# ivargr/kmer_mapper

Measured on AMD Instinct MI355X. Metric: M k-mers mapped/sec (whole node), k=31 150bp reads, higher is better.
Workload: dtype u64

## Files before the change

### kmer_mapper_amd/csrc/kmm.hip

```cpp
#include <hip/hip_runtime.h>

#include <cstdarg>
#include <cstdint>
#include <cstdio>
#include <cstdlib>
#include <chrono>
#include <cstring>
#include <memory>
#include <mutex>
#include <string>
#include <thread>
#include <utility>
#include <vector>

#include "kmm.h"

namespace {

thread_local std::string g_err;

int fail(int code, const char *fmt, ...)
{
    char buf[1024];
    va_list ap;
// ... 539 lines not shown
    if (w < 0 || w > 13 || ix->modulo >= (1ull << 31))
        return false;
    const uint64_t PF = (ix->modulo + (1ull << w) - 1) >> w;
    if (PF > (uint64_t)maxf * maxf)
        return false;
    int lg = 0;
    while ((1ull << lg) < PF)
        ++lg;
    int f2 = (lg + 1) / 2;
    bool for_filter = false;
    int occ_shift = 0;
    if (ix->rx_filter && w + f2 > P2F_LOGBITS) {
        const double load = ix->rx_S ? (double)ix->rx_S / (double)ix->modulo : 0.5;
        for (int gs = 0; gs <= 2 && !for_filter; ++gs) {
            const int fb = P2F_LOGBITS + gs - w;
            if (fb < 0 || load * (double)(1 << gs) > 0.75)
                continue;
            if (((PF + (1ull << fb) - 1) >> fb) <= (uint64_t)RX_MAXF && fb <= 9) {
                f2 = fb;
                occ_shift = gs;
                for_filter = true;
            }
        }
    }
    if (f2_force >= 0) {
        f2 = f2_force;
        occ_shift = w + f2 > P2F_LOGBITS ? w + f2 - P2F_LOGBITS : 0;
    }
    const uint64_t max_quo = ~0ull / ix->modulo;
    auto fits = [&](int sh) { return sh == 0 || (sh < 64 && (max_quo >> (64 - sh)) == 0); };
    while (f2 > 0 && !fits(w + f2))
        --f2;
    if (!fits(w + f2))
        return false;
    const uint64_t F2 = 1ull << f2, F1 = (PF + F2 - 1) / F2;
    if (F2 > (uint64_t)maxf || F1 > (uint64_t)(for_filter ? RX_MAXF : maxf))
        return false;
    ix->rx_w = w;
    ix->rx_f2 = f2;
    ix->rx_occ_shift = w + f2 > P2F_LOGBITS ? w + f2 - P2F_LOGBITS : 0;
    (void)occ_shift;
    ix->rx_PF = (uint32_t)PF;
    ix->rx_F1 = (uint32_t)F1;
    ix->rx_F2 = (uint32_t)F2;
    return true;
}

bool rx_filter_active(const kmm_index *ix)
{
    const int sh = ix->rx_w + ix->rx_f2;
    return ix->rx_filter && ix->rx_occ && sh - ix->rx_occ_shift >= 5 && ix->rx_occ_shift <= 2;
}

bool use_radix(const kmm_index *ix, int64_t units)
{
    if (!ix->rx_ok || ix->path == 1)
        return false;
    return ix->path == 2 || ix->rx_ecnt_acc || units >= ix->rx_min_units;
}

size_t align256(size_t x) { return (x + 255) & ~(size_t)255; }

template <int MODE>
int launch_rx(kmm_index *ix, const ReadsView &rv, const uint64_t *kmers_in, int64_t n_in, int k, int max_freq,
              int also_rc)
{
    const IndexView iv = view_of(ix);
    const int64_t units = MODE == MODE_KMERS ? n_in : rv.total;
    const int64_t n_src_total = MODE == MODE_PACKED ? (rv.n_reads + 2 * (int64_t)rv.pk_rpt - 1) / (2 * (int64_t)rv.pk_rpt)
                                                    : (units + RX_B - 1) / RX_B;
    const uint32_t X = also_rc ? 2u : 1u;
    const uint32_t F1 = ix->rx_F1, F2 = ix->rx_F2;
    int64_t n_sub = 1, max_src = 0;
    static const bool verbose = getenv("KMM_VERBOSE") != nullptr;
    const auto t_0 = std::chrono::steady_clock::now();
    if (ix->rx_sub_cap_eff > 0 && ++ix->rx_sub_cap_eff_age >= 16)
        ix->rx_sub_cap_eff = 0;
    int64_t cap = ix->rx_sub_cap_eff > 0 && ix->rx_sub_cap_eff < ix->rx_sub_cap ? ix->rx_sub_cap_eff : ix->rx_sub_cap;
    for (;;) {
        const int64_t cap_src = (cap / RX_B) / X > 0 ? (cap / RX_B) / X : 1;
        n_sub = (n_src_total + cap_src - 1) / cap_src;
        max_src = n_sub ? (n_src_total + n_sub - 1) / n_sub : cap_src;
        const size_t NBm = (size_t)max_src * X, chunks_m = (NBm + RX_CH - 1) / RX_CH, items_m = NBm + F1 + 1;
        const size_t meta = align256(NBm * (F1 + 1) * 2) + align256((size_t)F1 * (NBm + 1) * 4) + align256((size_t)F1 * NBm * 2) +
                            align256(chunks_m * F1 * 4) + 3 * align256((size_t)(F1 + 1) * 4) + align256(items_m * 8) +
                            align256(items_m * (F2 + 1) * 2) + align256(items_m * (F2 + 1) * 2 + 256) + align256(64) + align256(2048);
        int rc = ix->dbg_rx_buf_limit && NBm * RX_B * 8 > (size_t)ix->dbg_rx_buf_limit ? (int)KMM_ERR_NOMEM
                                                                                         : ensure(ix->rx_meta, meta);
        if (rc == KMM_OK)
            rc = ensure(ix->rx_buf1, NBm * RX_B * 8);
        if (rc == KMM_OK)
            rc = ensure(ix->rx_buf2, items_m * RX_B * 8);
        if (rc == KMM_OK)
            break;
        if (rc != KMM_ERR_NOMEM || cap <= ((int64_t)1 << 28) || n_src_total <= 1)
            return rc;
        (void)hipGetLastError();
        (void)ix->rx_buf1.reset();
        (void)ix->rx_buf2.reset();
        const int64_t next_src = (n_src_total + n_sub) / (n_sub + 1);
        cap = next_src * RX_B * X;
        if (cap < ((int64_t)1 << 28))
            cap = (int64_t)1 << 28;
        ix->rx_sub_cap_eff = cap;
        ix->rx_sub_cap_eff_age = 0;
    }
    ix->rx_sub_cap_last = cap;
    const double ms_buffers = ms_since(t_0);
    for (int64_t s0 = 0; s0 < n_src_total; s0 += max_src) {
        const uint32_t n_src = (uint32_t)(n_src_total - s0 < max_src ? n_src_total - s0 : max_src);
        const uint32_t NB = n_src * X;
        const uint32_t chunks = (NB + RX_CH - 1) / RX_CH;
        const size_t max_items = (size_t)NB + F1 + 1;
        RxView rx;
        memset(&rx, 0, sizeof rx);
        rx.pstart = ix->rx_pstart; rx.pkeys = ix->rx_pkeys; rx.pfreq = ix->rx_pfreq; rx.ecnt = ix->rx_ecnt;
        rx.pstart16 = ix->rx_pstart16; rx.slice_e0 = ix->rx_slice_e0; rx.slice_fmax = ix->rx_slice_fmax;
        rx.occ = ix->rx_occ;
        rx.occ_shift = rx_filter_active(ix) ? ix->rx_occ_shift : 3;
        rx.p2f_k = NB / 2048u < 4u ? 4u : (NB / 2048u > (uint32_t)P2F_KMAX ? (uint32_t)P2F_KMAX : NB / 2048u);
        rx.w = ix->rx_w; rx.f2 = ix->rx_f2; rx.PF = ix->rx_PF; rx.F1 = F1; rx.F2 = F2;
        rx.NB = NB; rx.max_items = (uint32_t)max_items;
        size_t off = 0;
        auto carve = [&](size_t bytes) { const size_t o = off; off += align256(bytes); return o; };
        const size_t o_start1 = carve((size_t)NB * (F1 + 1) * 2), o_P1T = carve((size_t)F1 * (NB + 1) * 4),
                     o_S1T = carve((size_t)F1 * NB * 2), o_csum = carve((size_t)chunks * F1 * 4),
                     o_T1 = carve((size_t)F1 * 4), o_ib = carve((size_t)(F1 + 1) * 4), o_wb = carve((size_t)(F1 + 1) * 4),
                     o_desc = carve(max_items * 8), o_start2 = carve(max_items * (F2 + 1) * 2), o_start2T = carve(max_items * (F2 + 1) * 2 + 256),
                     o_ctrl = carve(64),
                     o_queue = carve(2048);
        KMMCHK(ensure(ix->rx_meta, off));
        KMMCHK(ensure(ix->rx_buf1, (size_t)NB * RX_B * 8));
        KMMCHK(ensure(ix->rx_buf2, max_items * RX_B * 8));
        uint8_t *m = (uint8_t *)ix->rx_meta.p;
        rx.start1 = (uint16_t *)(m + o_start1); rx.P1T = (uint32_t *)(m + o_P1T); rx.S1T = (uint16_t *)(m + o_S1T);
        rx.csum = (uint32_t *)(m + o_csum); rx.T1 = (uint32_t *)(m + o_T1); rx.item_base = (uint32_t *)(m + o_ib);
        rx.work_base = (uint32_t *)(m + o_wb); rx.item_desc = (uint2 *)(m + o_desc);
        rx.start2 = (uint16_t *)(m + o_start2); rx.start2T = (uint16_t *)(m + o_start2T);
        rx.ctrl = (uint32_t *)(m + o_ctrl);
        rx.queue = (unsigned long long *)(m + o_queue);
        rx.buf1 = (uint64_t *)ix->rx_buf1.p;
        rx.buf2 = (uint64_t *)ix->rx_buf2.p;
#if RX_PROBE_ANY
        KMMCHK(ensure(ix->rx_probe, max_items * RX_B * 8));
        rx.probe = (uint64_t *)ix->rx_probe.p;
#endif
        ix->dbg_T1 = rx.T1; ix->dbg_item_base = rx.item_base; ix->dbg_start1 = rx.start1; ix->dbg_F1 = F1; ix->dbg_NB = NB;
        HIPCHK(hipMemsetAsync(m + o_ctrl, 0, align256(64) + 2048, ix->stream));
        ScopedTimer tm;
        KMMCHK(tm.begin(ix, KMM_KERNEL_RX_P1));
        static const int p1_per_cu = getenv("KMM_RX_P1_GRID_PER_CU") ? atoi(getenv("KMM_RX_P1_GRID_PER_CU")) : 8;
        const int64_t g1cap = (int64_t)ix->n_cu * (p1_per_cu > 0 ? p1_per_cu : 8);
        const dim3 g1((unsigned)(n_src < g1cap ? n_src : g1cap));
        const int64_t tile0 = s0 * (RX_B / (MODE == MODE_RECORDS ? 1024 : 4096));
        const uint64_t *src_kmers = kmers_in ? kmers_in + s0 * RX_B : nullptr;
        constexpr bool CAN_C2 = MODE == MODE_PACKED || MODE == MODE_UNIFORM || MODE == MODE_GENERAL;
        if (rv.codes2 && !CAN_C2)
            return fail(KMM_ERR_INTERNAL, "2-bit code input reaches pass 1 through the flat-read modes only");
        if constexpr (CAN_C2) {
            if (rv.codes2 && also_rc)
                hipLaunchKernelGGL((k_rx_p1<MODE, true, true>), g1, dim3(RX_NT), 0, ix->stream, rv, src_kmers, n_in - s0 * RX_B,
                                   iv, rx, k, tile0, n_src);
            else if (rv.codes2)
                hipLaunchKernelGGL((k_rx_p1<MODE, false, true>), g1, dim3(RX_NT), 0, ix->stream, rv, src_kmers, n_in - s0 * RX_B,
                                   iv, rx, k, tile0, n_src);
        }
        if (rv.codes2) {
        } else if (also_rc)
            hipLaunchKernelGGL((k_rx_p1<MODE, true>), g1, dim3(RX_NT), 0, ix->stream, rv, src_kmers, n_in - s0 * RX_B,
                               iv, rx, k, tile0, n_src);
        else
            hipLaunchKernelGGL((k_rx_p1<MODE, false>), g1, dim3(RX_NT), 0, ix->stream, rv, src_kmers, n_in - s0 * RX_B,
                               iv, rx, k, tile0, n_src);
        HIPCHK(hipGetLastError());
        KMMCHK(tm.end());
        KMMCHK(tm.begin(ix, KMM_KERNEL_RX_SCAN));
        hipLaunchKernelGGL(k_rx_colsum, dim3(chunks), dim3(256), 0, ix->stream, rx);
        hipLaunchKernelGGL(k_rx_chunkscan, dim3(F1), dim3(256), 0, ix->stream, rx, chunks);
        hipLaunchKernelGGL(k_rx_tables, dim3(1), dim3(512), 0, ix->stream, rx);
        hipLaunchKernelGGL(k_rx_colscan, dim3(chunks, (F1 + 255) / 256), dim3(256), 0, ix->stream, rx);
        HIPCHK(hipGetLastError());
        KMMCHK(tm.end());
        KMMCHK(tm.begin(ix, KMM_KERNEL_RX_P2));
        if (ix->rx_filter) {
            const bool flt = rx_filter_active(ix), small = F2 <= 128;
            auto kern = flt ? (small ? k_rx_p2f<true, true> : k_rx_p2f<true, false>)
                            : (small ? k_rx_p2f<false, true> : k_rx_p2f<false, false>);
            hipLaunchKernelGGL(kern, dim3(ix->n_cu), dim3(P2F_NT), 0, ix->stream, iv, rx);
        } else {
            hipLaunchKernelGGL(k_rx_p2, dim3(ix->n_cu * ix->rx_grid_per_cu), dim3(RX_NT), 0, ix->stream, iv, rx);
        }
        HIPCHK(hipGetLastError());
        KMMCHK(tm.end());
        KMMCHK(tm.begin(ix, KMM_KERNEL_RX_SCAN));
        hipLaunchKernelGGL(k_rx_tr2, dim3((unsigned)((max_items + RX_TR2 - 1) / RX_TR2)), dim3(256), 0, ix->stream, rx);
        HIPCHK(hipGetLastError());
        KMMCHK(tm.end());
        KMMCHK(tm.begin(ix, KMM_KERNEL_RX_P3));
        const bool p16 = ix->rx_pstart16 != nullptr;
        if (ix->rx_w > 12 && ix->rx_fits_small && p16)
            hipLaunchKernelGGL((k_rx_p3<RX_WMAX_BIG, RX_ECAP, 4, uint16_t, RX_SUBCAP3, true>), dim3(ix->n_cu * ix->rx_grid_per_cu),
                               dim3(RX_NT), 0, ix->stream, iv, rx, max_freq);
        else if (ix->rx_w > 12 && ix->rx_fits_small && ix->rx_max_slice <= 65535u)
            hipLaunchKernelGGL((k_rx_p3<RX_WMAX_BIG, RX_ECAP, 4, uint16_t>), dim3(ix->n_cu * ix->rx_grid_per_cu), dim3(RX_NT),
                               0, ix->stream, iv, rx, max_freq);
        else if (ix->rx_w > 12 && ix->rx_fits_mid && p16 && !getenv("KMM_RX_NO_MID"))
            hipLaunchKernelGGL((k_rx_p3<RX_WMAX_BIG, RX_ECAP_MID, 4, uint16_t, 1024, true>), dim3(ix->n_cu * ix->rx_grid_per_cu),
                               dim3(RX_NT), 0, ix->stream, iv, rx, max_freq);
        else if (ix->rx_w > 12 && ix->rx_fits_mid && ix->rx_max_slice <= 65535u && !getenv("KMM_RX_NO_MID"))
            hipLaunchKernelGGL((k_rx_p3<RX_WMAX_BIG, RX_ECAP_MID, 4, uint16_t, 1024>), dim3(ix->n_cu * ix->rx_grid_per_cu),
                               dim3(RX_NT), 0, ix->stream, iv, rx, max_freq);
        else if (ix->rx_w > 12)
            hipLaunchKernelGGL((k_rx_p3<RX_WMAX_BIG, RX_ECAP_BIG, 2, uint32_t>), dim3(ix->n_cu), dim3(RX_NT), 0, ix->stream,
                               iv, rx, max_freq);
        else if (ix->rx_w <= 12 && p16)
            hipLaunchKernelGGL((k_rx_p3<RX_WMAX, RX_ECAP, 4, uint16_t, RX_SUBCAP3, true>), dim3(ix->n_cu * ix->rx_grid_per_cu),
                               dim3(RX_NT), 0, ix->stream, iv, rx, max_freq);
        else
            hipLaunchKernelGGL((k_rx_p3<RX_WMAX, RX_ECAP, 4, uint32_t>), dim3(ix->n_cu * ix->rx_grid_per_cu), dim3(RX_NT), 0,
                               ix->stream, iv, rx, max_freq);
        HIPCHK(hipGetLastError());
        KMMCHK(tm.end());
        ix->ecnt_dirty = true;
        ix->rx_unchecked = true;
    }
    ix->n_radix_batches++;
    if (verbose && ms_since(t_0) > 20.0)
        fprintf(stderr, "libkmm: radix passes of %lld positions: %.2f ms for the batch buffers (%zu + %zu + %zu bytes), %.2f ms to issue %lld "
                "sub-batch(es)\n", (long long)units, ms_buffers, ix->rx_meta.cap, ix->rx_buf1.cap, ix->rx_buf2.cap, ms_since(t_0) - ms_buffers,
                (long long)n_sub);
    return KMM_OK;
}

int rx_flush(kmm_index *ix)
{
    if (!ix->ecnt_dirty)
        return KMM_OK;
    ScopedTimer tm;
    KMMCHK(tm.begin(ix, KMM_KERNEL_RX_FLUSH));
    if (ix->rx_norder && !ix->rx_ecnt_acc && ix->rx_flush_sorted) {
        hipLaunchKernelGGL(k_rx_flush_sorted, dim3(ix->n_cu * 8), dim3(256), 0, ix->stream, view_of(ix), ix->rx_ecnt,
                           ix->rx_norder, ix->rx_nnode, ix->rx_S);
        HIPCHK(hipMemsetAsync(ix->rx_ecnt, 0, (size_t)ix->rx_S * 4, ix->stream));
    } else {
        hipLaunchKernelGGL(k_rx_flush, dim3(ix->n_cu * 8), dim3(256), 0, ix->stream, view_of(ix), ix->rx_ecnt,
                           ix->rx_pnodes, ix->rx_S, ix->rx_ecnt_acc);
    }
    HIPCHK(hipGetLastError());
    KMMCHK(tm.end());
    ix->ecnt_dirty = false;
    return KMM_OK;
}

template <int MODE>
int launch_map_reads(kmm_index *ix, const ReadsView &rv, int k, int max_freq, int also_rc)
{
    const int64_t n_tiles = (rv.total + TILE_T - 1) / TILE_T;
    const bool radix = MODE == MODE_RECORDS ? false : use_radix(ix, rv.total);
    if (!radix) {
        KMMCHK(ensure_direct(ix));
        ix->n_direct_batches++;
        const IndexView iv = view_of(ix);
        ScopedTimer tm;
// ... 3329 lines not shown
```

### kmer_mapper_amd/csrc/kmm_radix.hpp

```cpp
#pragma once
#include <type_traits>

constexpr int RX_NT = 512;
constexpr int RX_B = 8192;
constexpr int RX_KPT = RX_B / RX_NT;
constexpr int RX_MAXF = 512;
#ifndef RX_CHV
#define RX_CHV 256
#endif
constexpr int RX_CH = RX_CHV;
constexpr int RX_IC = 1024;
#ifndef RX_LPR2V
#define RX_LPR2V 16
#endif
constexpr int RX_LPR = RX_LPR2V;
constexpr int RX_NG = RX_NT / RX_LPR;
#ifndef RX_RB1
#define RX_RB1 4
#endif
#ifndef RX_RB2
#define RX_RB2 8
#endif
constexpr int RX_SUBCAP = 1024;
#ifndef RX_SUBCAP3V
#define RX_SUBCAP3V 3072
#endif
constexpr int RX_SUBCAP3 = RX_SUBCAP3V;
#ifndef RX_LPR3
#define RX_LPR3 16
#endif
constexpr bool RX_P3_LINECUT = false;
constexpr int RX_LPR_P3 = RX_LPR3;
constexpr int RX_NG3 = RX_NT / RX_LPR_P3;
#ifndef RX_U3
#define RX_U3 8
#endif
constexpr int RX_U = RX_U3;
#ifndef RX_P3_GROUP
#define RX_P3_GROUP 4
#endif
constexpr int RX_G3 = RX_P3_GROUP;
#ifndef RX_U2V
#define RX_U2V 8
#endif
constexpr int RX_U2 = RX_U2V;
#ifdef RX_NT_LOADS
#define RX_LOAD2(p) __builtin_nontemporal_load(p)
#define RX_LOAD3(p) __builtin_nontemporal_load(p)
#else
#define RX_LOAD2(p) (*(p))
#define RX_LOAD3(p) (*(p))
#endif
constexpr int RX_WMAX = 4096;
constexpr int RX_ECAP = 4096;
constexpr int RX_WMAX_BIG = 8192;
constexpr int RX_ECAP_BIG = 8192;
constexpr int RX_ECAP_MID = 4608;
constexpr uint32_t RX_FILTERED = 0x80000000u;
enum { MODE_KMERS = 3 };

struct RxView {
    const uint16_t *pstart16;
    const uint32_t *slice_e0;
    const uint16_t *slice_fmax;
    const uint32_t *pstart;
    const uint64_t *pkeys;
    const uint16_t *pfreq;
    uint32_t *ecnt;
    const uint32_t *occ;
    uint32_t p2f_k;
    int w, f2;
    int occ_shift;
    uint32_t PF, F1, F2;
    uint32_t NB;
    uint32_t max_items;
    uint64_t *buf1, *buf2;
    uint16_t *start1;
    uint32_t *P1T;
    uint16_t *S1T;
    uint32_t *csum;
    uint32_t *T1;
    uint32_t *item_base;
    uint32_t *work_base;
    uint2 *item_desc;
    uint16_t *start2;
    uint16_t *start2T;
    uint32_t *ctrl;
    unsigned long long *queue;
    uint64_t *probe;
};

#ifndef RX_PROBE_P1W
#define RX_PROBE_P1W 0
#endif
#ifndef RX_PROBE_P2R
#define RX_PROBE_P2R 0
#endif
#ifndef RX_PROBE_P2W
#define RX_PROBE_P2W 0
#endif
#ifndef RX_PROBE_P3R
#define RX_PROBE_P3R 0
#endif
#define RX_PROBE_ANY (RX_PROBE_P1W || RX_PROBE_P2R || RX_PROBE_P2W || RX_PROBE_P3R)

__device__ __forceinline__ uint64_t rx_pack(const IndexView &iv, int sh, uint64_t q, uint32_t *coarse)
{
    uint32_t h;
    const uint64_t quo = fastdiv_m31(q, (uint32_t)iv.modulo, iv.magic, &h);
    *coarse = h >> sh;
    return (quo << sh) | (uint64_t)(h & ((1u << sh) - 1u));
}

__device__ __forceinline__ uint2 rx_pair(const uint32_t *s_in, int c0, int n)
{
    const uint2 p = *reinterpret_cast<const uint2 *>(s_in + c0);
    return make_uint2(c0 < n ? p.x : 0u, c0 + 1 < n ? p.y : 0u);
}

template <bool ONEBAR>
__device__ __forceinline__ uint32_t rx_scan256(const uint32_t *s_in, uint32_t *s_out, int n, uint32_t *s_wave, const int tid)
{
    if (ONEBAR) {
    (void)s_wave;
    const int lane = tid & 63;
    const int wave = __builtin_amdgcn_readfirstlane(tid >> 6);
    if (wave < 4) {
        const uint32_t v = tid < n ? s_in[tid] : 0u;
        const uint32_t inc = wave_scan_incl(v);
        uint32_t before = 0;
        for (int x = 0; x < wave; ++x) {
            const uint32_t t = x * 64 + lane < n ? s_in[x * 64 + lane] : 0u;
            before += (uint32_t)__builtin_amdgcn_readlane((int)wave_scan_incl(t), 63);
        }
        if (tid < n)
            s_out[tid] = before + inc - v;
        if (tid == 255)
            s_out[n] = before + inc;
    }
    __syncthreads();
    return s_out[n];
    }
    const int lane = tid & 63, wave = tid >> 6;
    const uint32_t v = tid < n ? s_in[tid] : 0u;
    const uint32_t inc = wave_scan_incl(v);
    if (wave < 4 && lane == 63)
        s_wave[wave] = inc;
    __syncthreads();
    const uint32_t total = s_wave[0] + s_wave[1] + s_wave[2] + s_wave[3];
    if (tid < n) {
        uint32_t base = 0;
        for (int x = 0; x < wave; ++x)
            base += s_wave[x];
        s_out[tid] = base + inc - v;
    }
    if (tid == 0)
        s_out[n] = total;
    __syncthreads();
    return total;
}
// ... 418 lines not shown
        lookups += (uint32_t)__popc(valid) * X;
        RX_PT(0);
        if (RC) {
            uint64_t x[RX_KPT];
            auto fwd = [&](int i) {
                uint32_t c;
                x[i] = rx_pack(iv, sh, q[i], &c);
                return ((valid >> i) & 1u) ? c : spare;
            };
            rx_sort_emit<RX_RB1, true, true, RX_NT, true, decltype(fwd), RxNoHook, 0, true>(
                x, fwd, F1, sbuf, s_cnt, s_base, s_wave, rx.buf1 + (size_t)sb * 2 * RX_B,
                rx.start1 + (size_t)sb * 2 * (size_t)(F1 + 1) RX_PT_ARG2, RxNoHook(), RX_KPT, wave_s);
            auto rev = [&](int i) {
                uint32_t c;
                x[i] = rx_pack(iv, sh, revcomp(q[i], k), &c);
                return ((valid >> i) & 1u) ? c : spare;
            };
            rx_sort_emit<RX_RB1, MODE == MODE_KMERS, true, RX_NT, true, decltype(rev), RxNoHook, 0, true>(
                x, rev, F1, sbuf, s_cnt, s_base, s_wave, rx.buf1 + ((size_t)sb * 2 + 1) * RX_B,
                rx.start1 + ((size_t)sb * 2 + 1) * (size_t)(F1 + 1) RX_PT_ARG2, RxNoHook(), RX_KPT, wave_s);
        } else {
            uint32_t qlo = 0, qhi = 0, rem = 0;
            const uint32_t M32 = (uint32_t)iv.modulo, Ml = M32 & 0xFFFFu, Mh = M32 >> 16;
            const uint32_t nb = (uint32_t)((win.lo >> (2 * k)) | (win.hi << (64 - 2 * k)));
            uint4 e_nx = make_uint4(0u, 0u, 0u, 0u);
            auto fwd = [&](int i) {
                if constexpr (INCDIV && R == 1) {
                    const uint4 e = e_nx;
                    if (i + 1 < RX_KPT) {
                        uint32_t c = (nb >> (2 * i)) & 3u;
                        asm("" : "+v"(c) : "v"(rem));
                        e_nx = s_qr[c];
                    }
                    if (i == 0) {
                        const uint64_t quot = fastdiv_m31(win.lo & tc.kmask, M32, iv.magic, &rem);
                        qlo = (uint32_t)quot;
                        qhi = (uint32_t)(quot >> 32);
                    } else {
                        const uint32_t t = qlo & 3u;
                        uint32_t th = __umul24(t, Mh);
                        asm("" : "+v"(th));
                        const uint32_t y = ((__umul24(t, Ml) + rem) >> 2) + (th << 14);
                        const uint32_t r2 = y + e.x;
                        uint32_t nlo, nhi;
                        asm("v_alignbit_b32 %0, %3, %2, 2\n\t"
                            "v_lshrrev_b32 %1, 2, %3\n\t"
                            "v_cmp_le_u32 vcc, %6, %7\n\t"
                            "v_addc_co_u32 %0, vcc, %0, %4, vcc\n\t"
                            "v_addc_co_u32 %1, vcc, %1, %5, vcc"
                            : "=&v"(nlo), "=&v"(nhi)
                            : "v"(qlo), "v"(qhi), "v"(e.y), "v"(e.z), "s"(M32), "v"(r2)
                            : "vcc");
                        qlo = nlo;
                        qhi = nhi;
                        rem = r2 - M32 < r2 ? r2 - M32 : r2;
                    }
                    q[i] = ((((uint64_t)qhi << 32) | qlo) << sh) | (uint64_t)(rem & ((1u << sh) - 1u));
                    return ((valid >> i) & 1u) ? rem >> sh : spare;
                } else {
                    uint32_t c;
                    q[i] = rx_pack(iv, sh, q[i], &c);
                    return ((valid >> i) & 1u) ? c : spare;
                }
            };
            auto post = [&]() {
                if constexpr (STAGE_EARLY) {
                    if (sb + sb_step < sb_end)
                        tile_packed_stage<C2>(rv, tile_begin + ((int64_t)(sb + sb_step) * 2 + half), sm[half], ltid, pw[0]);
                }
            };
            rx_sort_emit<RX_RB1, MODE == MODE_KMERS, true, RX_NT, true, decltype(fwd), RxNoHook, 0, true, decltype(post)>(
                q, fwd, F1, sbuf, s_cnt, s_base, s_wave, rx.buf1 + (size_t)sb * RX_B,
                rx.start1 + (size_t)sb * (size_t)(F1 + 1) RX_PT_ARG2, RxNoHook(), RX_KPT, wave_s, post,
                RX_PROBE_P1W ? rx.probe + (size_t)sb * RX_B : nullptr, RX_PROBE_P1W);
        }
    }
#ifdef RX_PT_P1
    RX_PT_END(iv, 10);
#endif
    rx_stat_add(iv, 0, lookups);
    rx_stat_add(iv, KMM_STAT_RX_P1, lookups);
}

__global__ void __launch_bounds__(256) k_rx_colsum(RxView rx)
{
    const uint32_t F1 = rx.F1;
    const uint32_t b0 = blockIdx.x * RX_CH;
    const uint32_t b1 = b0 + RX_CH < rx.NB ? b0 + RX_CH : rx.NB;
    const size_t ld = F1 + 1;
    for (uint32_t c = threadIdx.x; c < F1; c += 256) {
        const uint16_t *p = rx.start1 + (size_t)b0 * ld + c;
        uint32_t sum = 0, b = b0;
        for (; b + 8 <= b1; b += 8, p += 8 * ld) {
            uint32_t lo[8], hi[8];
#pragma unroll
            for (int u = 0; u < 8; ++u) {
                lo[u] = p[u * ld];
                hi[u] = p[u * ld + 1];
            }
#pragma unroll
            for (int u = 0; u < 8; ++u)
                sum += hi[u] - lo[u];
        }
        for (; b < b1; ++b, p += ld)
            sum += (uint32_t)p[1] - (uint32_t)p[0];
        rx.csum[(size_t)blockIdx.x * F1 + c] = sum;
    }
}

__device__ __forceinline__ uint32_t scan256_excl(uint32_t v, uint32_t *s_wave4, uint32_t *total)
{
    const int lane = threadIdx.x & 63, wave = threadIdx.x >> 6;
    const uint32_t inc = wave_scan_incl(v);
    __syncthreads();
    if (lane == 63)
        s_wave4[wave] = inc;
    __syncthreads();
    uint32_t base = 0;
    for (int x = 0; x < wave; ++x)
        base += s_wave4[x];
    *total = s_wave4[0] + s_wave4[1] + s_wave4[2] + s_wave4[3];
    return base + inc - v;
}

__global__ void __launch_bounds__(256) k_rx_chunkscan(RxView rx, uint32_t n_chunks)
{
    __shared__ uint32_t s_wave4[4];
    const uint32_t c = blockIdx.x, F1 = rx.F1;
    uint32_t carry = 0;
    for (uint32_t base = 0; base < n_chunks; base += 256) {
        const uint32_t ch = base + threadIdx.x;
        const uint32_t v = ch < n_chunks ? rx.csum[(size_t)ch * F1 + c] : 0u;
        uint32_t tot;
        const uint32_t ex = scan256_excl(v, s_wave4, &tot);
        if (ch < n_chunks)
            rx.csum[(size_t)ch * F1 + c] = carry + ex;
        carry += tot;
    }
    if (threadIdx.x == 0) {
        rx.T1[c] = carry;
        rx.P1T[(size_t)c * (rx.NB + 1) + rx.NB] = carry;
    }
}

__device__ __forceinline__ uint32_t scan512_excl(uint32_t v, uint32_t *s_wave8, uint32_t *total)
{
    const int lane = threadIdx.x & 63, wave = threadIdx.x >> 6;
    const uint32_t inc = wave_scan_incl(v);
    __syncthreads();
    if (lane == 63)
        s_wave8[wave] = inc;
    __syncthreads();
    uint32_t base = 0, tot = 0;
    for (int x = 0; x < 8; ++x) {
        base += x < wave ? s_wave8[x] : 0u;
        tot += s_wave8[x];
    }
    *total = tot;
    return base + inc - v;
}

__global__ void __launch_bounds__(512) k_rx_tables(RxView rx)
{
    static_assert(RX_MAXF <= 512, "one thread per coarse partition");
    __shared__ uint32_t s_wave8[8];
    const uint32_t c = threadIdx.x, F1 = rx.F1;
    const uint32_t run = c < F1 ? rx.T1[c] : 0u;
    const uint32_t n_items = c < F1 ? (run + RX_B - 1) / RX_B : 0u;
    const uint32_t rows = (n_items + RX_IC - 1) / RX_IC;
    uint32_t tot_items, tot_rows;
    const uint32_t ib = scan512_excl(n_items, s_wave8, &tot_items);
    const uint32_t wb = scan512_excl(rows, s_wave8, &tot_rows);
    uint32_t jmax = n_items;
#pragma unroll
    for (int d = 32; d > 0; d >>= 1) {
        const uint32_t o = __shfl_xor(jmax, d);
        jmax = o > jmax ? o : jmax;
    }
    __syncthreads();
    if ((threadIdx.x & 63) == 0)
        s_wave8[threadIdx.x >> 6] = jmax;
    __syncthreads();
    if (c < F1) {
        rx.item_base[c] = ib;
        rx.work_base[c] = wb;
    }
    if (c == 0) {
        uint32_t m = s_wave8[0];
        for (int x = 1; x < 8; ++x)
            m = s_wave8[x] > m ? s_wave8[x] : m;
        rx.item_base[F1] = tot_items;
        rx.work_base[F1] = tot_rows;
        rx.ctrl[0] = tot_items;
        rx.ctrl[1] = tot_rows;
        rx.ctrl[2] = m;
    }
}

__global__ void __launch_bounds__(256) k_rx_colscan(RxView rx)
{
    constexpr int TB = 32, CW = 256;
    __shared__ uint32_t tP[CW][TB + 1];
    __shared__ uint16_t tS[CW][TB + 2];
    const uint32_t F1 = rx.F1, NB = rx.NB;
    const uint32_t b0 = blockIdx.x * RX_CH;
    const uint32_t b1 = b0 + RX_CH < NB ? b0 + RX_CH : NB;
    const size_t ld = F1 + 1;
    const uint32_t lane = threadIdx.x & 63, wave = threadIdx.x >> 6;
    {
    const uint32_t cb = blockIdx.y * CW;
    const uint32_t c = cb + threadIdx.x;
    const uint32_t nc = F1 - cb < (uint32_t)CW ? F1 - cb : (uint32_t)CW;
    uint32_t run = c < F1 ? rx.csum[(size_t)blockIdx.x * F1 + c] : 0u;
    const uint32_t ib = c < F1 ? rx.item_base[c] : 0u;
    for (uint32_t t0 = b0; t0 < b1; t0 += TB) {
        const uint32_t nb = b1 - t0 < (uint32_t)TB ? b1 - t0 : (uint32_t)TB;
        if (c < F1) {
            const uint16_t *p = rx.start1 + (size_t)t0 * ld + c;
            uint32_t lo[TB], hi[TB];
#pragma unroll
            for (int u = 0; u < TB; ++u) {
                lo[u] = (uint32_t)u < nb ? p[u * ld] : 0u;
                hi[u] = (uint32_t)u < nb ? p[u * ld + 1] : 0u;
            }
#pragma unroll
            for (int u = 0; u < TB; ++u) {
                const uint32_t cnt = hi[u] - lo[u];
                tP[threadIdx.x][u] = run;
                tS[threadIdx.x][u] = (uint16_t)lo[u];
                if (cnt) {
                    uint32_t m = (run + RX_B - 1) / RX_B;
                    while ((uint64_t)m * RX_B < (uint64_t)run + cnt) {
                        rx.item_desc[ib + m] = make_uint2(t0 + u, c);
                        ++m;
                    }
                }
                run += cnt;
            }
        }
        __syncthreads();
        const uint32_t bi = lane & 31;
        for (uint32_t cc = wave * 2 + (lane >> 5); cc < nc; cc += 8) {
            if (bi < nb) {
                rx.P1T[(size_t)(cb + cc) * (NB + 1) + t0 + bi] = tP[cc][bi];
                rx.S1T[(size_t)(cb + cc) * NB + t0 + bi] = tS[cc][bi];
            }
        }
        __syncthreads();
    }
    }
}

constexpr int RX_TR2 = 32;
__global__ void __launch_bounds__(256) k_rx_tr2(RxView rx)
{
    __shared__ uint16_t tile[RX_TR2][RX_MAXF + 2];
    const uint32_t n_items = rx.ctrl[0], cols = rx.F2 + 1;
    const uint32_t i0 = blockIdx.x * RX_TR2;
    if (i0 >= n_items)
        return;
    const uint32_t ni = n_items - i0 < (uint32_t)RX_TR2 ? n_items - i0 : (uint32_t)RX_TR2;
    for (uint32_t e = threadIdx.x; e < ni * cols; e += 256)
        tile[e / cols][e % cols] = rx.start2[(size_t)i0 * cols + e];
    __syncthreads();
    const uint32_t it = threadIdx.x % RX_TR2, c0 = threadIdx.x / RX_TR2;
    if (it < ni)
        for (uint32_t col = c0; col < cols; col += 256 / RX_TR2)
            rx.start2T[(size_t)col * rx.max_items + i0 + it] = tile[it][col];
}

__global__ void __launch_bounds__(RX_NT, 4) k_rx_p2(IndexView iv, RxView rx)
{
    __shared__ uint64_t sbuf[RX_B];
    __shared__ uint32_t sub_src[RX_SUBCAP];
    __shared__ uint32_t sub_meta[RX_SUBCAP], s_wave8[2][RX_NT / 64];
    __shared__ __attribute__((aligned(8))) uint32_t s_cnt[RX_MAXF + 2 + 64];
    __shared__ uint32_t s_base[RX_MAXF + 1], s_wave[4];
    __shared__ uint32_t s_idx;
    const int tid = threadIdx.x, grp = tid / RX_LPR, lg = tid % RX_LPR;
    const uint32_t NB = rx.NB;
    uint32_t gathered = 0;
    uint32_t scan_flip = 0;
    const uint32_t spare = rx_spare_key();
    const int F2 = (int)rx.F2;
    const uint32_t cs = (rx.F1 + 7u) / 8u, limit = rx.ctrl[2] * cs;
    const uint32_t home = rx_xcc_id();
    if (tid <= F2)
        s_cnt[tid] = 0;
    if (tid == 0)
        s_cnt[RX_NT] = 0;
    struct Item {
        uint32_t valid, c, item, b0, lo, hi;
    };
    struct RunDesc {
        uint32_t vs, ve, st;
    };
    auto describe = [&](uint32_t sub, uint32_t idx) {
        Item d;
        d.valid = 0; d.c = 0; d.item = 0; d.b0 = 0; d.lo = 0; d.hi = 0;
        if (idx >= limit)
            return d;
        const uint32_t cj = idx / cs, cc = sub * cs + idx % cs;
        if (cc >= rx.F1)
            return d;
        const uint32_t ib = rx.item_base[cc];
        if (cj >= rx.item_base[cc + 1] - ib)
            return d;
        d.valid = 1;
        d.c = cc;
        d.item = ib + cj;
        d.b0 = rx.item_desc[d.item].x;
        d.lo = cj * RX_B;
        const uint32_t Tc = rx.T1[cc];
        d.hi = Tc - d.lo < (uint32_t)RX_B ? Tc : d.lo + RX_B;
        return d;
    };
    auto run_desc = [&](const Item &d, uint32_t bb) {
        RunDesc r;
        r.vs = 0xFFFFFFFFu; r.ve = 0xFFFFFFFFu; r.st = 0;
        const uint32_t b = bb + tid;
        if (d.valid && b < NB) {
            const uint32_t *P = rx.P1T + (size_t)d.c * (NB + 1);
            r.vs = P[b];
            r.ve = P[b + 1];
            r.st = rx.S1T[(size_t)d.c * NB + b];
        }
        return r;
    };
    RX_PT_DECL;
    for (uint32_t turn = 0; turn < 8u; ++turn) {
    const uint32_t sub = (home + turn) & 7u;
    uint32_t nxt = limit;
    if (tid == 0)
        nxt = rx_pop(rx.queue, sub, limit);
    if (tid == 0)
        s_idx = nxt;
    __syncthreads();
    uint32_t idx = s_idx;
    __syncthreads();
    if (idx >= limit)
        continue;
    if (tid == 0)
        nxt = rx_pop(rx.queue, sub, limit);
    Item it = describe(sub, idx);
    RunDesc rd = run_desc(it, it.b0);
    for (;;) {
        RX_PT(0);
        const uint32_t lo = it.lo, hi = it.hi, n = hi - lo;
        if (it.valid) {
            for (uint32_t bb = it.b0;; bb += RX_NT) {
                if (bb != it.b0)
                    rd = run_desc(it, bb);
                const uint32_t b = bb + tid;
                const uint32_t vs = rd.vs < hi ? rd.vs : hi;
                const bool live = vs < hi;
                const uint32_t ve = live ? rd.ve : vs;
                const uint32_t st = live ? rd.st : 0u;
                const uint32_t from = vs > lo ? vs : lo, to = ve < hi ? ve : hi;
                const uint32_t len = live && to > from ? to - from : 0u;
                const uint64_t src = (uint64_t)b * RX_B + st + (from - vs);
                uint32_t n_sub;
                const uint32_t last_more = (tid == RX_NT - 1 && live && ve < hi) ? 0x80000000u : 0u;
                const uint32_t pre = rx_scan_threads(rx_n_pieces<RX_LPR, true>(len, src) | last_more, s_wave8, scan_flip, &n_sub);
                const bool more = n_sub >> 31;
                n_sub &= 0x7FFFFFFFu;
                RX_PT(1);
                for (uint32_t win = 0; win < n_sub; win += RX_SUBCAP) {
                    rx_list_subruns<RX_LPR, true>(pre, len, src, from - lo, win, sub_src, sub_meta);
                    const uint32_t nw = n_sub - win < (uint32_t)RX_SUBCAP ? n_sub - win : (uint32_t)RX_SUBCAP;
                    rx_pad_list<RX_NG * RX_U2>(nw, sub_src, sub_meta);
                    __syncthreads();
                    for (uint32_t j0 = grp; j0 < nw; j0 += RX_NG * RX_U2) {
                        uint64_t x[RX_U2];
                        uint32_t meta[RX_U2], so[RX_U2];
#pragma unroll
                        for (int u = 0; u < RX_U2; ++u) {
                            meta[u] = sub_meta[j0 + u * RX_NG];
                            so[u] = sub_src[j0 + u * RX_NG];
                        }
#pragma unroll
                        for (int u = 0; u < RX_U2; ++u) {
                            const uint32_t rel = (uint32_t)lg - ((meta[u] >> 6) & 63u);
                            x[u] = rel < (meta[u] & 63u) ? RX_LOAD2(rx.buf1 + ((size_t)so[u] + lg)) : 0ull;
                        }
#pragma unroll
                        for (int u = 0; u < RX_U2; ++u) {
                            const uint32_t rel = (uint32_t)lg - ((meta[u] >> 6) & 63u);
                            if (rel < (meta[u] & 63u))
                                sbuf[(meta[u] >> 12) + rel] = x[u];
                        }
                    }
                    if (more || win + RX_SUBCAP < n_sub)
                        __syncthreads();
                }
                if (!more)
                    break;
            }
        }
        if (tid == 0)
            s_idx = nxt;
        __syncthreads();
        const uint32_t idx_n = s_idx;
        if (tid == 0 && idx_n < limit)
            nxt = rx_pop(rx.queue, sub, limit);
        const Item it_n = describe(sub, idx_n);
        RunDesc rd_n;
        rd_n.vs = 0xFFFFFFFFu; rd_n.ve = 0xFFFFFFFFu; rd_n.st = 0;
        if (it.valid) {
// ... 29 lines not shown
    }
#ifndef RX_PT_P1
    RX_PT_END(iv, 10);
#endif
    rx_stat_add(iv, 2, gathered);
}

__device__ __forceinline__ uint32_t rx_fold2(uint32_t x)
{
    x = (x | (x >> 1)) & 0x55555555u;
    x = (x | (x >> 1)) & 0x33333333u;
    x = (x | (x >> 2)) & 0x0F0F0F0Fu;
    x = (x | (x >> 4)) & 0x00FF00FFu;
    return (x | (x >> 8)) & 0x0000FFFFu;
}
__device__ __forceinline__ uint32_t rx_fold4(uint32_t x)
{
    x = (x | (x >> 1) | (x >> 2) | (x >> 3)) & 0x11111111u;
    x = (x | (x >> 3)) & 0x03030303u;
    x = (x | (x >> 6)) & 0x000F000Fu;
    return (x | (x >> 12)) & 0xFFu;
}

constexpr int P2F_NT = 1024;
constexpr int P2F_KPT = RX_B / P2F_NT;
constexpr int P2F_KMAX = 64;
constexpr int P2F_LOGBITS = 19;

template <bool FILTER, bool FSMALL>
__global__ void __launch_bounds__(P2F_NT) k_rx_p2f(IndexView iv, RxView rx)
{
    __shared__ uint32_t s_bits[(1 << P2F_LOGBITS) / 32];
    __shared__ uint64_t sbuf[RX_B];
    __shared__ uint32_t t_vs[P2F_NT + 64];
    __shared__ uint32_t t_off[P2F_NT];
    __shared__ uint16_t t_aux[RX_B / 64 + 1];
    __shared__ uint32_t t_last;
    __shared__ uint32_t t_sbits[2][RX_B / 32];
    __shared__ uint32_t t_empty[2];
    __shared__ __attribute__((aligned(8))) uint32_t s_cnt2[2][RX_MAXF + 2 + 64];
    __shared__ uint32_t s_base[RX_MAXF + 1], s_wave[4];
    __shared__ uint32_t s_b0[P2F_KMAX];
    __shared__ uint32_t s_idx;
    const int tid = threadIdx.x, lane = tid & 63;
    const uint32_t wave = (uint32_t)__builtin_amdgcn_readfirstlane(tid >> 6);
    const uint32_t NB = rx.NB;
    const int F2 = (int)rx.F2, w = rx.w;
    const uint32_t bmask = (1u << (rx.w + rx.f2)) - 1u;
    const uint32_t gs = (uint32_t)rx.occ_shift;
    constexpr bool nofilt = !FILTER;
    const uint32_t nwords = nofilt ? 0u : (((uint32_t)F2 << w) >> gs) / 32u;
    const uint32_t spare = rx_spare_key();
    uint32_t gathered = 0, dropped = 0;
    const uint32_t cs = (rx.F1 + 7u) / 8u;
    const uint32_t P2F_K = rx.p2f_k;
    const uint32_t limit = ((rx.ctrl[2] + P2F_K - 1u) / P2F_K) * cs;
    const uint32_t home = rx_xcc_id();
    if (tid <= F2)
        s_cnt2[0][tid] = s_cnt2[1][tid] = 0;
    RX_PT_DECL;

    struct RunDesc {
        uint32_t vs, ve, st;
    };
    for (uint32_t turn = 0; turn < 8u; ++turn) {
    const uint32_t sub = (home + turn) & 7u;
    for (;;) {
        if (tid == 0)
            s_idx = rx_pop(rx.queue, sub, limit);
        __syncthreads();
        const uint32_t idx = s_idx;
        __syncthreads();
        if (idx >= limit)
            break;
        const uint32_t cu = idx / cs, cc = sub * cs + idx % cs;
        if (cc >= rx.F1)
            continue;
        const uint32_t ib = rx.item_base[cc], n_items_c = rx.item_base[cc + 1] - ib;
        if (cu * P2F_K >= n_items_c)
            continue;
        const uint32_t j0 = cu * P2F_K;
        const uint32_t n_it = n_items_c - j0 < P2F_K ? n_items_c - j0 : P2F_K;
        const uint32_t Tc = rx.T1[cc];
        const uint32_t *P = rx.P1T + (size_t)cc * (NB + 1);
        const uint16_t *S = rx.S1T + (size_t)cc * NB;
        if ((uint32_t)tid < n_it)
            s_b0[tid] = rx.item_desc[ib + j0 + tid].x;
        if (nofilt) {
        } else if (gs == 0) {
            const uint4 *src = reinterpret_cast<const uint4 *>(rx.occ + (size_t)cc * nwords);
            uint4 *dst = reinterpret_cast<uint4 *>(s_bits);
            for (uint32_t i = tid; i < nwords / 4u; i += P2F_NT)
                dst[i] = src[i];
            for (uint32_t i = (nwords & ~3u) + tid; i < nwords; i += P2F_NT)
                s_bits[i] = rx.occ[(size_t)cc * nwords + i];
        } else {
            const uint32_t *src = rx.occ + (((size_t)cc * nwords) << gs);
            for (uint32_t i = tid; i < nwords; i += P2F_NT) {
                uint32_t o = 0;
                if (gs == 1) {
                    const uint2 v = *reinterpret_cast<const uint2 *>(src + 2 * (size_t)i);
                    o = rx_fold2(v.x) | (rx_fold2(v.y) << 16);
                } else {
                    const uint4 v = *reinterpret_cast<const uint4 *>(src + 4 * (size_t)i);
                    o = rx_fold4(v.x) | (rx_fold4(v.y) << 8) | (rx_fold4(v.z) << 16) | (rx_fold4(v.w) << 24);
                }
                s_bits[i] = o;
            }
        }
        if (tid < 2 * (RX_B / 32))
            (&t_sbits[0][0])[tid] = 0u;
        if (tid < 2)
            t_empty[tid] = 0u;
        __syncthreads();

        auto item_lo = [&](uint32_t j) { return (j0 + j) * (uint32_t)RX_B; };
        auto item_n = [&](uint32_t j) {
            const uint32_t lo = (j0 + j) * (uint32_t)RX_B;
            return Tc - lo < (uint32_t)RX_B ? Tc - lo : (uint32_t)RX_B;
        };
        auto load_desc = [&](uint32_t bb) {
            RunDesc r;
            const uint32_t b = bb + tid;
            r.vs = 0xFFFFFFFFu; r.ve = 0xFFFFFFFFu; r.st = 0;
            if (b < NB) {
                r.vs = P[b];
                r.ve = P[b + 1];
                r.st = S[b];
            }
            return r;
        };
        auto put_table = [&](const RunDesc &r, uint32_t lo, uint32_t hi, int mb = -1) {
            if (mb >= 0 && r.vs != 0xFFFFFFFFu && r.vs > lo && r.vs < hi) {
                if (r.ve > r.vs)
                    atomicOr(&t_sbits[mb][(r.vs - lo) >> 5], 1u << ((r.vs - lo) & 31u));
                else
                    t_empty[mb] = 1u;
            }
            t_vs[tid] = r.vs;
            t_off[tid] = (uint32_t)tid * RX_B + r.st - r.vs;
            if (tid == P2F_NT - 1) {
                t_vs[P2F_NT] = r.ve;
                if (r.ve < hi)
                    t_last = P2F_NT - 1;
            }
            const uint32_t from = r.vs > lo ? r.vs : lo, to = r.ve < hi ? r.ve : hi;
            if (r.vs != 0xFFFFFFFFu && from < to) {
                for (uint32_t a = (from - lo + 63u) >> 6; lo + (a << 6) < to; ++a)
                    t_aux[a] = (uint16_t)tid;
                if (to == hi)
                    t_last = (uint32_t)tid;
            }
        };
        auto fill = [&](auto merge_tag, uint32_t bb, uint32_t lo, uint32_t n, uint32_t c_lo, uint32_t c_hi,
                        uint64_t (&x)[P2F_KPT], int mb = -1) {
            constexpr bool MERGE = decltype(merge_tag)::value;
            const uint32_t c_end = lo + n < c_hi ? lo + n : c_hi;
            const uint32_t a0 = wave * 8u;
            uint32_t av = 0;
            {
                const uint32_t pa = lo + ((a0 + (uint32_t)lane) << 6);
                const uint32_t ia = a0 + ((uint32_t)lane <= 8u ? (uint32_t)lane : 8u);
                const uint32_t aux = t_aux[ia];
                av = pa < c_lo ? 0u : (pa < c_end ? aux : t_last);
            }
            uint32_t A[P2F_KPT + 1];
#pragma unroll
            for (int i = 0; i <= P2F_KPT; ++i)
// ... 721 lines not shown
```

Before: 169,600.

## Restructure radix column-scan with 64x64 tiles and padded transposed tables

Pads the transposed P1T/S1T tables to a leading dimension rounded up to 64 so that tiled writes start line-aligned. Rewrites k_rx_colscan to process 64-column by 64-row tiles with four waves that split the rows, software-prefetch the next tile, derive counts through a lane shuffle instead of a second load, and scan across waves through shared memory. k_rx_colsum now loads each start1 entry once and differences adjacent columns through shared memory, launched with one thread per column. The goal is to cut redundant global loads and uncoalesced stores in the scan stage. The cost is more shared-memory synchronisation and slightly larger metadata buffers.

```diff
diff --git a/kmer_mapper_amd/csrc/kmm.hip b/kmer_mapper_amd/csrc/kmm.hip
--- a/kmer_mapper_amd/csrc/kmm.hip
+++ b/kmer_mapper_amd/csrc/kmm.hip
@@ -645,7 +645,8 @@
         n_sub = (n_src_total + cap_src - 1) / cap_src;
         max_src = n_sub ? (n_src_total + n_sub - 1) / n_sub : cap_src;
         const size_t NBm = (size_t)max_src * X, chunks_m = (NBm + RX_CH - 1) / RX_CH, items_m = NBm + F1 + 1;
-        const size_t meta = align256(NBm * (F1 + 1) * 2) + align256((size_t)F1 * (NBm + 1) * 4) + align256((size_t)F1 * NBm * 2) +
+        const size_t ldTm = (NBm + RX_TT) / RX_TT * RX_TT;
+        const size_t meta = align256(NBm * (F1 + 1) * 2) + align256((size_t)F1 * ldTm * 4) + align256((size_t)F1 * ldTm * 2) +
                             align256(chunks_m * F1 * 4) + 3 * align256((size_t)(F1 + 1) * 4) + align256(items_m * 8) +
                             align256(items_m * (F2 + 1) * 2) + align256(items_m * (F2 + 1) * 2 + 256) + align256(64) + align256(2048);
         int rc = ix->dbg_rx_buf_limit && NBm * RX_B * 8 > (size_t)ix->dbg_rx_buf_limit ? (int)KMM_ERR_NOMEM
@@ -684,10 +685,11 @@
         rx.p2f_k = NB / 2048u < 4u ? 4u : (NB / 2048u > (uint32_t)P2F_KMAX ? (uint32_t)P2F_KMAX : NB / 2048u);
         rx.w = ix->rx_w; rx.f2 = ix->rx_f2; rx.PF = ix->rx_PF; rx.F1 = F1; rx.F2 = F2;
         rx.NB = NB; rx.max_items = (uint32_t)max_items;
+        rx.ldT = (NB + RX_TT) / RX_TT * RX_TT;
         size_t off = 0;
         auto carve = [&](size_t bytes) { const size_t o = off; off += align256(bytes); return o; };
-        const size_t o_start1 = carve((size_t)NB * (F1 + 1) * 2), o_P1T = carve((size_t)F1 * (NB + 1) * 4),
-                     o_S1T = carve((size_t)F1 * NB * 2), o_csum = carve((size_t)chunks * F1 * 4),
+        const size_t o_start1 = carve((size_t)NB * (F1 + 1) * 2), o_P1T = carve((size_t)F1 * rx.ldT * 4),
+                     o_S1T = carve((size_t)F1 * rx.ldT * 2), o_csum = carve((size_t)chunks * F1 * 4),
                      o_T1 = carve((size_t)F1 * 4), o_ib = carve((size_t)(F1 + 1) * 4), o_wb = carve((size_t)(F1 + 1) * 4),
                      o_desc = carve(max_items * 8), o_start2 = carve(max_items * (F2 + 1) * 2), o_start2T = carve(max_items * (F2 + 1) * 2 + 256),
                      o_ctrl = carve(64),
@@ -738,10 +740,10 @@
         HIPCHK(hipGetLastError());
         KMMCHK(tm.end());
         KMMCHK(tm.begin(ix, KMM_KERNEL_RX_SCAN));
-        hipLaunchKernelGGL(k_rx_colsum, dim3(chunks), dim3(256), 0, ix->stream, rx);
+        hipLaunchKernelGGL(k_rx_colsum, dim3(chunks), dim3((F1 + 63) / 64 * 64), 0, ix->stream, rx);
         hipLaunchKernelGGL(k_rx_chunkscan, dim3(F1), dim3(256), 0, ix->stream, rx, chunks);
         hipLaunchKernelGGL(k_rx_tables, dim3(1), dim3(512), 0, ix->stream, rx);
-        hipLaunchKernelGGL(k_rx_colscan, dim3(chunks, (F1 + 255) / 256), dim3(256), 0, ix->stream, rx);
+        hipLaunchKernelGGL(k_rx_colscan, dim3((F1 + RX_TT - 1) / RX_TT, chunks), dim3(256), 0, ix->stream, rx);
         HIPCHK(hipGetLastError());
         KMMCHK(tm.end());
         KMMCHK(tm.begin(ix, KMM_KERNEL_RX_P2));
diff --git a/kmer_mapper_amd/csrc/kmm_radix.hpp b/kmer_mapper_amd/csrc/kmm_radix.hpp
--- a/kmer_mapper_amd/csrc/kmm_radix.hpp
+++ b/kmer_mapper_amd/csrc/kmm_radix.hpp
@@ -76,6 +76,7 @@
     uint32_t max_items;
     uint64_t *buf1, *buf2;
     uint16_t *start1;
+    uint32_t ldT;
     uint32_t *P1T;
     uint16_t *S1T;
     uint32_t *csum;
@@ -660,30 +661,33 @@
     rx_stat_add(iv, KMM_STAT_RX_P1, lookups);
 }
 
-__global__ void __launch_bounds__(256) k_rx_colsum(RxView rx)
-{
-    const uint32_t F1 = rx.F1;
+__global__ void __launch_bounds__(RX_MAXF) k_rx_colsum(RxView rx)
+{
+    __shared__ uint32_t s_e[RX_MAXF];
+    const uint32_t F1 = rx.F1, j = threadIdx.x;
     const uint32_t b0 = blockIdx.x * RX_CH;
     const uint32_t b1 = b0 + RX_CH < rx.NB ? b0 + RX_CH : rx.NB;
     const size_t ld = F1 + 1;
-    for (uint32_t c = threadIdx.x; c < F1; c += 256) {
-        const uint16_t *p = rx.start1 + (size_t)b0 * ld + c;
-        uint32_t sum = 0, b = b0;
-        for (; b + 8 <= b1; b += 8, p += 8 * ld) {
-            uint32_t lo[8], hi[8];
-#pragma unroll
-            for (int u = 0; u < 8; ++u) {
-                lo[u] = p[u * ld];
-                hi[u] = p[u * ld + 1];
-            }
-#pragma unroll
-            for (int u = 0; u < 8; ++u)
-                sum += hi[u] - lo[u];
+    uint32_t e = 0;
+    if (j < F1) {
+        const uint16_t *p = rx.start1 + (size_t)b0 * ld + j + 1;
+        uint32_t b = b0;
+        for (; b + 16 <= b1; b += 16, p += 16 * ld) {
+            uint32_t x[16];
+#pragma unroll
+            for (int u = 0; u < 16; ++u)
+                x[u] = p[u * ld];
+#pragma unroll
+            for (int u = 0; u < 16; ++u)
+                e += x[u];
         }
         for (; b < b1; ++b, p += ld)
-            sum += (uint32_t)p[1] - (uint32_t)p[0];
-        rx.csum[(size_t)blockIdx.x * F1 + c] = sum;
-    }
+            e += p[0];
+    }
+    s_e[j] = e;
+    __syncthreads();
+    if (j < F1)
+        rx.csum[(size_t)blockIdx.x * F1 + j] = e - (j ? s_e[j - 1] : 0u);
 }
 
 __device__ __forceinline__ uint32_t scan256_excl(uint32_t v, uint32_t *s_wave4, uint32_t *total)
@@ -717,7 +721,7 @@
     }
     if (threadIdx.x == 0) {
         rx.T1[c] = carry;
-        rx.P1T[(size_t)c * (rx.NB + 1) + rx.NB] = carry;
+        rx.P1T[(size_t)c * rx.ldT + rx.NB] = carry;
     }
 }
 
@@ -775,57 +779,76 @@
     }
 }
 
+constexpr int RX_TT = 64;
+static_assert(RX_CH % RX_TT == 0, "tiles of a chunk start line-aligned");
 __global__ void __launch_bounds__(256) k_rx_colscan(RxView rx)
 {
-    constexpr int TB = 32, CW = 256;
-    __shared__ uint32_t tP[CW][TB + 1];
-    __shared__ uint16_t tS[CW][TB + 2];
+    constexpr int T = RX_TT, RPW = RX_TT / 4;
+    __shared__ uint32_t tP[T][T + 1];
+    __shared__ uint16_t tS[T][T + 2];
+    __shared__ uint32_t s_tot[4][T];
     const uint32_t F1 = rx.F1, NB = rx.NB;
-    const uint32_t b0 = blockIdx.x * RX_CH;
+    const size_t ld = F1 + 1, ldT = rx.ldT;
+    const uint32_t lane = threadIdx.x & 63, wave = threadIdx.x >> 6;
+    const uint32_t c0 = blockIdx.x * T, c = c0 + lane;
+    const uint32_t nc = F1 - c0 < (uint32_t)T ? F1 - c0 : (uint32_t)T;
+    const uint32_t b0 = blockIdx.y * RX_CH;
     const uint32_t b1 = b0 + RX_CH < NB ? b0 + RX_CH : NB;
-    const size_t ld = F1 + 1;
-    const uint32_t lane = threadIdx.x & 63, wave = threadIdx.x >> 6;
-    {
-    const uint32_t cb = blockIdx.y * CW;
-    const uint32_t c = cb + threadIdx.x;
-    const uint32_t nc = F1 - cb < (uint32_t)CW ? F1 - cb : (uint32_t)CW;
-    uint32_t run = c < F1 ? rx.csum[(size_t)blockIdx.x * F1 + c] : 0u;
+    const bool ext = c0 + T <= F1;
+    uint32_t run = c < F1 ? rx.csum[(size_t)blockIdx.y * F1 + c] : 0u;
     const uint32_t ib = c < F1 ? rx.item_base[c] : 0u;
-    for (uint32_t t0 = b0; t0 < b1; t0 += TB) {
-        const uint32_t nb = b1 - t0 < (uint32_t)TB ? b1 - t0 : (uint32_t)TB;
-        if (c < F1) {
-            const uint16_t *p = rx.start1 + (size_t)t0 * ld + c;
-            uint32_t lo[TB], hi[TB];
-#pragma unroll
-            for (int u = 0; u < TB; ++u) {
-                lo[u] = (uint32_t)u < nb ? p[u * ld] : 0u;
-                hi[u] = (uint32_t)u < nb ? p[u * ld + 1] : 0u;
-            }
-#pragma unroll
-            for (int u = 0; u < TB; ++u) {
-                const uint32_t cnt = hi[u] - lo[u];
-                tP[threadIdx.x][u] = run;
-                tS[threadIdx.x][u] = (uint16_t)lo[u];
-                if (cnt) {
-                    uint32_t m = (run + RX_B - 1) / RX_B;
-                    while ((uint64_t)m * RX_B < (uint64_t)run + cnt) {
-                        rx.item_desc[ib + m] = make_uint2(t0 + u, c);
-                        ++m;
-                    }
-                }
-                run += cnt;
-            }
-        }
+    uint32_t lo[RPW], nx = 0;
+    auto load = [&](uint32_t t0) {
+        const uint32_t r0 = t0 + wave * RPW;
+        const uint16_t *p = rx.start1 + (size_t)r0 * ld;
+#pragma unroll
+        for (int u = 0; u < RPW; ++u)
+            lo[u] = c <= F1 && r0 + u < b1 ? p[u * ld + c] : 0u;
+        nx = ext && lane < (uint32_t)RPW && r0 + lane < b1 ? p[lane * ld + c0 + T] : 0u;
+    };
+    load(b0);
+    for (uint32_t t0 = b0; t0 < b1; t0 += T) {
+        uint32_t cur[RPW];
+#pragma unroll
+        for (int u = 0; u < RPW; ++u)
+            cur[u] = lo[u];
+        const uint32_t cnx = nx;
+        if (t0 + T < b1)
+            load(t0 + T);
+        uint32_t cnt[RPW], tot = 0;
+#pragma unroll
+        for (int u = 0; u < RPW; ++u) {
+            const uint32_t up = (uint32_t)__shfl_down((int)cur[u], 1);
+            const uint32_t hi = lane == 63 ? (uint32_t)__builtin_amdgcn_readlane((int)cnx, u) : up;
+            cnt[u] = c < F1 ? hi - cur[u] : 0u;
+            tot += cnt[u];
+        }
+        s_tot[wave][lane] = tot;
         __syncthreads();
-        const uint32_t bi = lane & 31;
-        for (uint32_t cc = wave * 2 + (lane >> 5); cc < nc; cc += 8) {
-            if (bi < nb) {
-                rx.P1T[(size_t)(cb + cc) * (NB + 1) + t0 + bi] = tP[cc][bi];
-                rx.S1T[(size_t)(cb + cc) * NB + t0 + bi] = tS[cc][bi];
-            }
+        uint32_t v = run;
+#pragma unroll
+        for (int x = 0; x < 4; ++x) {
+            const uint32_t t = s_tot[x][lane];
+            v += (uint32_t)x < wave ? t : 0u;
+            run += t;
+        }
+#pragma unroll
+        for (int u = 0; u < RPW; ++u) {
+            const uint32_t r = wave * RPW + u;
+            tP[lane][r] = v;
+            tS[lane][r] = (uint16_t)cur[u];
+            const uint64_t m = ((uint64_t)v + RX_B - 1) / RX_B;
+            if (m * RX_B < (uint64_t)v + cnt[u])
+                rx.item_desc[ib + (uint32_t)m] = make_uint2(t0 + r, c);
+            v += cnt[u];
         }
         __syncthreads();
-    }
+        const uint32_t nb = b1 - t0 < (uint32_t)T ? b1 - t0 : (uint32_t)T;
+        if (lane < nb)
+            for (uint32_t r = wave; r < nc; r += 4) {
+                rx.P1T[(size_t)(c0 + r) * ldT + t0 + lane] = tP[r][lane];
+                rx.S1T[(size_t)(c0 + r) * ldT + t0 + lane] = tS[r][lane];
+            }
     }
 }
 
@@ -898,10 +921,10 @@
         r.vs = 0xFFFFFFFFu; r.ve = 0xFFFFFFFFu; r.st = 0;
         const uint32_t b = bb + tid;
         if (d.valid && b < NB) {
-            const uint32_t *P = rx.P1T + (size_t)d.c * (NB + 1);
+            const uint32_t *P = rx.P1T + (size_t)d.c * rx.ldT;
             r.vs = P[b];
             r.ve = P[b + 1];
-            r.st = rx.S1T[(size_t)d.c * NB + b];
+            r.st = rx.S1T[(size_t)d.c * rx.ldT + b];
         }
         return r;
     };
@@ -1097,8 +1120,8 @@
         const uint32_t j0 = cu * P2F_K;
         const uint32_t n_it = n_items_c - j0 < P2F_K ? n_items_c - j0 : P2F_K;
         const uint32_t Tc = rx.T1[cc];
-        const uint32_t *P = rx.P1T + (size_t)cc * (NB + 1);
-        const uint16_t *S = rx.S1T + (size_t)cc * NB;
+        const uint32_t *P = rx.P1T + (size_t)cc * rx.ldT;
+        const uint16_t *S = rx.S1T + (size_t)cc * rx.ldT;
         if ((uint32_t)tid < n_it)
             s_b0[tid] = rx.item_desc[ib + j0 + tid].x;
         if (nofilt) {
```

New measurement: 171,600 (median of 6 runs). About the same (+1.2%).
